# xuhao1/TaichiSLAM

Hardware: AMD Instinct MI355X
Metric: depth-frames/s integrated (640x480->512^3 TSDF) (higher is better)
Workload: dtype f16 storage / f32 + int64 fixed-point arithmetic; 1 GPU; BASELINE configs[1]: single 640x480 u16 depth stream (sphere room r=3 m, 1 deg/frame) -> DenseTSDF 512^3 / 2 cm, recast_step 2, max_ray 5 m; one stream+submap per GPU

## Files before the change

### taichislam_amd/csrc/tsl_integrate.hip

```cpp
#include "tsl_tsdf.hpp"
#include <hip/hip_ext.h>

namespace tsl {

#ifdef TSL_TIMING
#define TSL_T0() const int _wv = (blockIdx.x * (int)blockDim.x + (int)threadIdx.x) >> 6
#define TSL_TICK(F, k) do { long long _n = wall_clock64(); if (lane_id() == 0 && _wv < 16384) (F).dbg[_wv * 16 + (k)] = _n; } while (0)
#else
#define TSL_T0() do {} while (0)
#define TSL_TICK(F, k) do {} while (0)
#endif

#define SCATTER_TILE 4096

struct RayRegs { float pf0, pf1, pf2, d0, d1, d2, P0, P1, P2, w; long long qden; int n; };

__device__ __forceinline__ uint32_t wave_min_u32(uint32_t v)
{
    for (int d = 32; d > 0; d >>= 1) { const uint32_t o = (uint32_t)__shfl_xor((int)v, d); v = o < v ? o : v; }
    return v;
}
__device__ __forceinline__ RayRegs make_ray(const uint4 rec, int n, const FrameParams& P)
{
    RayRegs R;
// ... 426 lines not shown
    if (i < nact) {
        b = F.act_b[i];
        v = F.bhist[b];
        int vq[TSL_NB];
#pragma unroll
        for (int q = 0; q < TSL_NB; ++q) { vq[q] = q < B.n ? B.f[q].bhist[b] : 0; if (vq[q] > 0) tm |= 1 << q; wb += vq[q]; }
        if (wb > unit_max) { tmp = tm; }
        else if (wb > unit_half) {
            int acc = 0;
#pragma unroll
            for (int q = 0; q < TSL_NB; ++q) if ((tm >> q) & 1) { if (2 * acc < wb) { tmu |= 1 << q; wu += vq[q]; } else tmp |= 1 << q; acc += vq[q]; }
        } else { tmu = tm; wu = wb; }
        if (tmu && (tmu & -tmu) == (1 << y)) ucls = plan_class(wu);
        if (((tmp >> y) & 1) && v > 0) { np = (v + psegs - 1) / psegs; pcls = plan_class((v + np - 1) / np); }
    }
    const int off = block_reserve_n(&F.counters[3], v);
    const int s0 = block_reserve_n(&B.f[0].counters[HDR_SLAB], np);
    int p0 = 0, u0 = 0;
    for (int c = 0; c < PLAN_NCLS; ++c) {
        const int q = block_reserve_n(&F.counters[HDR_PARTS + c], pcls == c ? np : 0); if (pcls == c) p0 = q;
        const int u = block_reserve_n(&B.f[0].counters[HDR_UNITS + c], ucls == c ? 1 : 0); if (ucls == c) u0 = u;
    }
    if (i < nact) {
        F.boffset[b] = off;
        F.bnseg[b] = v;
        const int pool = (np || ucls >= 0) ? pool_claim<false>(M, B.p[y]->slot, b) : -1;
        if (ucls >= 0) {
            if (u0 < B.f[0].unit_cap) B.f[0].unit_tab[(size_t)ucls * B.f[0].unit_cap + u0] = make_int4(b, wu, pool, tmu);
            else for (int q = 0; q < B.n; ++q) if ((tm >> q) & 1) frame_fail(M, B.f[q], 2);
        }
        if (np && pool >= 0) {
            if ((tmp & -tmp) == (1 << y)) {
                const int hi = __hip_atomic_fetch_add(&B.f[0].counters[HDR_HEAVY], 1, __ATOMIC_RELAXED, __HIP_MEMORY_SCOPE_AGENT);
                if (hi < B.f[0].max_frame_bricks) B.f[0].heavy_tab[hi] = make_int4(b, pool, tmp, 0);
                else for (int q = 0; q < B.n; ++q) if ((tm >> q) & 1) frame_fail(M, B.f[q], 2);
            }
// ... 546 lines not shown
#pragma unroll
        for (int k = 0; k < VP; ++k) if (changed[k]) {
            tw[l0 + k * 256] = cur[k];
            if ((first[k] >> 16) == 0u) obs[l0 + k * 256] = 1;
        }
    }
}

int check_variant2(tsl_tsdf* m)
{
    TSL_REQUIRE(m->F.max_frame_bricks <= 4096 && m->P.max_steps_f < (float)(1 << SEG_J_BITS) && m->F.max_points < (1 << STG_RAY_BITS) && m->nb3 < (1 << 24) && 3 * m->pcl_bits <= H_BLOCK_SHIFT,
                "variant 2: ray too long / too many points / too many bricks for the segment key (use variant 1)");
    return TSL_OK;
}

int launch_segments(tsl_tsdf* m, const BatchDev& B, const FrameParams* hp, int total, hipStream_t st)
{
    const FrameParams& P = hp[0];
    if (P.variant != 2) return TSL_OK;
    const int iblocks = (int)(((int64_t)total * P.split + 255) / 256);
    prof_begin(m, TSL_K_SEGMENTS, st);
    if (P.group) hipLaunchKernelGGL(k_segments<true>, dim3(iblocks, B.n), dim3(256), 0, st, m->M, B);
    else hipLaunchKernelGGL(k_segments<false>, dim3(iblocks, B.n), dim3(256), 0, st, m->M, B);
    prof_end(m, st);
    int unit_max = m->unit_max <= m->unit_floor ? m->unit_max : std::max(m->unit_floor, (int)((long long)m->unit_max * B.n / TSL_NB));
    int unit_half = std::min(unit_max, m->unit_half <= 2048 ? m->unit_half : std::max(2048, (int)((long long)m->unit_half * B.n / TSL_NB)));
    if (P.seq && m->seq_impl) unit_max = unit_half = 1 << 30;
    prof_begin(m, TSL_K_BIN, st);
    hipLaunchKernelGGL(k_plan, dim3((B.f[0].max_frame_bricks + 255) / 256, B.n), dim3(256), 0, st, m->M, B, m->chunks * m->wg * m->spt, unit_max, unit_half);
    hipLaunchKernelGGL(k_scatter, dim3(256, B.n), dim3(256), 0, st, B);
    prof_end(m, st);
    return TSL_OK;
}

int launch_brick(tsl_tsdf* m, const BatchDev& B, const FrameParams& P, int kind, hipStream_t st, hipEvent_t start, hipEvent_t stop)
{
    const int bg = kind == 2 ? m->pgrid : (B.n <= 2 ? (m->bgrid + 1) / 2 : (kind == 1 ? m->ugrid : m->bgrid));
#define TSL_LAUNCH_IB(TEXV, FD) do { \
        if (m->wg == 512 && m->spt == 2 && !TEXV) hipExtLaunchKernelGGL((k_integrate_batch<false, FD, 512, 2, 4>), dim3((2 * m->ncu * bg + 99) / 100), dim3(512), 0, st, start, stop, 0, m->M, B, kind); \
// ... 41 lines not shown
```

### taichislam_amd/csrc/tsl_tsdf.hip

```cpp
#include "tsl_tsdf.hpp"
#include <rocprim/rocprim.hpp>
#include <algorithm>
#include <cmath>
#include <cstdio>
#include <cstdlib>
#include <cstring>
#include <mutex>

namespace tsl {

static thread_local std::string g_err;
void set_error(const std::string& s) { g_err = s; }

__device__ __forceinline__ uint32_t part1by2_32(uint32_t x)
{
    x &= 0x3ffu;
    x = (x ^ (x << 16)) & 0xff0000ffu;
    x = (x ^ (x << 8)) & 0x0300f00fu;
    x = (x ^ (x << 4)) & 0x030c30c3u;
    x = (x ^ (x << 2)) & 0x09249249u;
    return x;
}
__device__ __forceinline__ uint64_t part1by2_64(uint64_t x)
{
// ... 437 lines not shown
        uint4 v[4];
#pragma unroll
        for (int u = 0; u < 4; ++u) { const int j = i + u * 256; v[u] = j < n ? src[j] : make_uint4(0u, 0u, 0u, 0u); }
#pragma unroll
        for (int u = 0; u < 4; ++u) { const int j = i + u * 256; if (j < n) dst[j] = v[u]; }
    }
}

__global__ void k_set_params(ParamPack PP, SetPtrs S)
{
    if (threadIdx.x == 0) *S.p[blockIdx.x] = PP.p[blockIdx.x];
    S.header[blockIdx.x][threadIdx.x] = 0;
}

template <typename K>
static int enqueue_phase_a(tsl_tsdf* m, const BatchDev& B, const FrameParams* hp, hipStream_t sa)
{
    const int n = B.n;
    int total = 0, tiles = 0, any_points = 0, any_depth = 0;
    for (int q = 0; q < n; ++q) {
        total = hp[q].total > total ? hp[q].total : total;
        const int t = ((hp[q].ww + 15) / 16) * ((hp[q].hh + 15) / 16);
        if (hp[q].points) any_points = 1; else { any_depth = 1; tiles = t > tiles ? t : tiles; }
    }
    if (total <= 0) return TSL_OK;
    const FrameParams& P0 = hp[0];
    const int blocks = (total + 255) / 256;
    prof_begin(m, TSL_K_VOXELIZE, sa);
    if (any_points) hipLaunchKernelGGL(k_voxelize_points<K>, dim3(blocks, n), dim3(256), 0, sa, B);
    if (any_depth) hipLaunchKernelGGL(k_voxelize_depth<K>, dim3(tiles, n), dim3(256), 0, sa, B);
    prof_end(m, sa);
    if (!P0.group) {
        const FrameDev& F = B.f[0];
        prof_begin(m, TSL_K_SORT, sa);
        size_t tb = m->sort_temp_bytes;
        TSL_HIP(rocprim::radix_sort_pairs(m->fset[m->cur * TSL_NB].sort_temp, tb, reinterpret_cast<K*>(F.keys), reinterpret_cast<K*>(F.keys_s), F.vals, F.vals_s, (size_t)total, 0u, (unsigned)(3 * P0.pcl_bits + 1), sa));
        prof_end(m, sa);
        prof_begin(m, TSL_K_RAYS, sa);
        hipLaunchKernelGGL(k_build_rays<K>, dim3(blocks), dim3(256), 0, sa, B.p[0], F, (const K*)reinterpret_cast<K*>(F.keys_s));
        prof_end(m, sa);
    }
    return launch_segments(m, B, hp, total, sa);
}

template <typename K>
static int launch_batch_t(tsl_tsdf* m)
{
    const int n = m->npend;
    if (n == 0) return TSL_OK;
    m->npend = 0;
    (void)hipGetLastError();
    m->last_batch_n = n;
    const int bi = m->cur;
    BatchHost& H = m->batch[bi];
    const bool serial = m->overlap == 0;
    {
        const BatchHost& L = m->batch[(bi + TSL_NBATCH - 1) % TSL_NBATCH];
        if (!L.b_pending || hipEventQuery(L.b_done) == hipSuccess) { m->ramp = 0; ++m->dry_launches; } else if (m->ramp < 1000) ++m->ramp;
        m->shape_hash = (m->shape_hash ^ (uint32_t)n) * 16777619u;
    }
    hipStream_t sa = serial ? m->stream_ : H.st;
    const int ring = (int)(m->batch_seq % TSL_INFLIGHT);
    if (m->ring_upto[ring] > 0) {
        TSL_HIP(hipEventSynchronize(m->ring_ev[ring]));
        if (m->ring_upto[ring] > m->frames_consumed) m->frames_consumed = m->ring_upto[ring];
    }
#ifdef TSL_TEST_HOOKS
    static const bool fault_no_wait = std::getenv("TSL_FAULT_NO_BDONE_WAIT") != nullptr;
#else
    constexpr bool fault_no_wait = false;
#endif
    if (!serial && H.b_pending && !fault_no_wait) TSL_HIP(hipStreamWaitEvent(sa, H.b_done, 0));
    if (!serial && m->esdf_gate_set) {
        TSL_HIP(hipStreamWaitEvent(sa, m->esdf_gate_ev, 0));
        m->esdf_gate_mask |= 1u << (bi % TSL_NSTREAMS);
        if (m->esdf_gate_mask == (1u << TSL_NSTREAMS) - 1u) m->esdf_gate_set = false;
    }
    for (int k = 0; k < m->nproducers; ++k) {
        if (m->producers[k] == sa) continue;
        if (hipStreamQuery(m->producers[k]) == hipSuccess) continue;
        if (!m->in_ev[0]) for (auto& e : m->in_ev) TSL_HIP(hipEventCreateWithFlags(&e, hipEventDisableTiming));
        hipEvent_t e = m->in_ev[m->in_ev_next]; m->in_ev_next = (m->in_ev_next + 1) % 8;
        TSL_HIP(hipEventRecord(e, m->producers[k]));
        TSL_HIP(hipStreamWaitEvent(sa, e, 0));
    }
    m->nproducers = 0;
    BatchDev B; ParamPack PP;
    for (int q = 0; q < n; ++q) { FSet& S = m->fset[bi * TSL_NB + q]; B.f[q] = S.F; B.p[q] = S.Pd; PP.p[q] = m->pend[q]; }
    for (int q = n; q < TSL_NB; ++q) { B.f[q] = B.f[0]; B.p[q] = B.p[0]; PP.p[q] = PP.p[0]; }
    B.n = n;
    SetPtrs SP;
    for (int q = 0; q < TSL_NB; ++q) { SP.p[q] = const_cast<FrameParams*>(B.p[q]); SP.header[q] = reinterpret_cast<int*>(B.f[q].stats); }
    hipLaunchKernelGGL(k_set_params, dim3(n), dim3(64), 0, sa, PP, SP);
    {
        StageCopy C; int most = 0; bool any_host = false;
        for (int q = 0; q < TSL_NB; ++q) {
            FSet& S = m->fset[bi * TSL_NB + q];
            const bool on = q < n;
            C.src[2 * q] = static_cast<const uint4*>(S.pin_dev); C.dst[2 * q] = static_cast<uint4*>(S.stage_in); C.n16[2 * q] = on ? (int)((S.copy_in + 15) / 16) : 0;
            C.src[2 * q + 1] = reinterpret_cast<const uint4*>(static_cast<const char*>(S.pin_dev) + S.copy_tex_off); C.dst[2 * q + 1] = static_cast<uint4*>(S.stage_tex); C.n16[2 * q + 1] = on ? (int)((S.copy_tex + 15) / 16) : 0;
            most = std::max(most, std::max(C.n16[2 * q], C.n16[2 * q + 1]));
            any_host = any_host || C.n16[2 * q] || C.n16[2 * q + 1];
            if (on) { S.copy_in = 0; S.copy_tex = 0; }
        }
        if (any_host) {
            prof_begin(m, TSL_K_VOXELIZE, sa);
            hipLaunchKernelGGL(k_stage_host, dim3(std::min(64, (most + 1023) / 1024), 2 * n), dim3(256), 0, sa, C);
            prof_end(m, sa);
            if (!serial) { TSL_HIP(hipEventRecord(H.c_done, sa)); H.c_recorded = true; }
        }
    }
    if (m->phases & 1) { int rc = enqueue_phase_a<K>(m, B, m->pend, sa); if (rc) return rc; }
    const bool seq_bricks = m->pend[0].seq && m->seq_impl && m->pend[0].variant == 2;
    if (seq_bricks && (m->phases & 1)) { int rc = launch_seq_group(m, B, m->pend, bi, sa); if (rc) return rc; }
    m->frames_issued += n;
    if (!serial) {
        TSL_HIP(hipEventRecord(H.a_done, sa)); H.a_recorded = true;
        TSL_HIP(hipStreamWaitEvent(m->stream_, H.a_done, 0));
    }
    bool any = false; for (int q = 0; q < n; ++q) any = any || m->pend[q].total > 0;
    const bool split = !serial && m->split_launch && (m->phases & 2) && m->pend[0].variant == 2 && !m->pend[0].seq && n > 2 && any;
    if (split) {
        hipEvent_t pa = nullptr, pb = nullptr;
        const bool timed = prof_slot(m, TSL_K_INTEGRATE, 0, &pa, &pb);
        int rc = launch_brick(m, B, m->pend[0], 2, sa, timed ? pa : nullptr, timed ? pb : nullptr);
        if (rc) return rc;
        TSL_HIP(hipEventRecord(H.p_done, sa));
// ... 51 lines not shown
template <int PICK>
static void pick_pixels(uint16_t* __restrict__ dst, const uint16_t* __restrict__ src, int n, int pick)
{
    if (PICK) { for (int i = 0; i < n; ++i) dst[i] = src[(size_t)i * PICK]; }
    else for (int i = 0; i < n; ++i) dst[i] = src[(size_t)i * pick];
}
static int stage_host(tsl_tsdf* m, int si, const void* in, size_t row_bytes, int rows, size_t src_pitch, const void* tex, size_t tex_bytes, void** in_dev, void** tex_dev,
                      int pick = 1)
{
    const int npick = pick > 1 ? (int)(row_bytes / sizeof(uint16_t)) / pick : 0;
    const size_t out_row = pick > 1 ? (size_t)npick * sizeof(uint16_t) : row_bytes;
    const size_t in_bytes = out_row * (size_t)rows;
    FSet& S = m->fset[si];
    BatchHost& H = m->batch[si / TSL_NB];
    if (m->overlap == 0) TSL_HIP(hipStreamSynchronize(m->stream_));
    else if (H.c_recorded) TSL_HIP(hipEventSynchronize(H.c_done));
    const size_t tex_off = (in_bytes + 255) & ~(size_t)255;
    const size_t need = tex_off + ((tex && tex_bytes) ? tex_bytes : 0) + 256;
    if (S.pin_bytes < need) {
        if (S.pin) (void)hipHostFree(S.pin);
        S.pin = nullptr; S.pin_bytes = 0; S.pin_dev = nullptr;
#ifdef TSL_TEST_HOOKS
        static const bool legacy = std::getenv("TSL_PIN_LEGACY") != nullptr;
#else
        constexpr bool legacy = false;
#endif
        TSL_HIP(hipHostMalloc(&S.pin, need + need / 4, legacy ? hipHostMallocMapped : (hipHostMallocMapped | hipHostMallocCoherent)));
        S.pin_bytes = need + need / 4;
        TSL_HIP(hipHostGetDevicePointer(&S.pin_dev, S.pin, 0));
    }
    char* pin = static_cast<char*>(S.pin);
// ... 108 lines not shown
    if (P.variant == 2) { int rc = check_variant2(m); if (rc) return rc; }
    P.input = xyz_dev ? xyz_dev : depth_dev; P.total = total; P.points = xyz_dev ? 1 : 0;
    {
        int lg = 10; while ((1ll << lg) < 2 * (long long)total) ++lg;
        P.hlog2 = lg < m->fset[0].F.hlog2 ? lg : m->fset[0].F.hlog2;
    }
    TSL_REQUIRE(!P.tex || P.variant == 2, "texture integration needs the brick-binned path (variant 2)");
    const int cap = batch_cap(m);
    { int si = 0; int rc = reserve_slot(m, P.points, &si); if (rc) return rc; }
    m->clean = false;
    m->pend_points = P.points;
    m->pend[m->npend] = P;
    m->pend[m->npend].group = (P.group && P.variant == 2) ? 1 : 0;
    m->last_set = m->cur * TSL_NB + m->npend;
    m->npend++;
    if (m->npend >= cap || (cap > 4 && m->ramp < m->ramp_batches && m->npend >= m->ramp_size)) return flush_pending(m);
    if (cap > 1 && m->adaptive) {
        const int last = (m->cur + TSL_NBATCH - 1) % TSL_NBATCH;
        const BatchHost& H = m->batch[last];
        if (!H.a_recorded || hipEventQuery(H.a_done) == hipSuccess) return flush_pending(m);
    }
    return TSL_OK;
}

static int sort_temp_size(tsl_tsdf* m, size_t* bytes)
{
    size_t a = 0, b = 0;
    TSL_HIP(rocprim::radix_sort_pairs(nullptr, a, (uint32_t*)nullptr, (uint32_t*)nullptr, (uint32_t*)nullptr, (uint32_t*)nullptr,
                                      (size_t)m->F.max_points, 0u, 32u, m->stream_));
    TSL_HIP(rocprim::radix_sort_pairs(nullptr, b, (uint64_t*)nullptr, (uint64_t*)nullptr, (uint32_t*)nullptr, (uint32_t*)nullptr,
                                      (size_t)m->F.max_points, 0u, 64u, m->stream_));
// ... 36 lines not shown
{
    int c = 0;
    hipError_t e = hipGetDeviceCount(&c);
    if (e != hipSuccess) { c = 0; }
    if (n) *n = c;
    return TSL_OK;
}

static int init_handle(tsl_tsdf* m, const tsl_tsdf_cfg* cfg, int device)
{
    m->cfg = *cfg; m->device = device; m->bytes = 0;
    (void)hipGetLastError();
    TSL_HIP(hipStreamCreateWithFlags(&m->stream_, hipStreamNonBlocking));
    m->overlap = TSL_NB; m->last_set = 0;
    for (auto& S : m->fset) { S.sort_temp = nullptr; S.header = nullptr; S.Pd = nullptr; S.stage_in = nullptr; S.stage_in_bytes = 0; S.stage_tex = nullptr; S.stage_tex_bytes = 0; S.pin = nullptr; S.pin_bytes = 0; S.pin_dev = nullptr; S.copy_in = S.copy_tex = S.copy_tex_off = 0; }
    for (auto& H : m->batch) { H.st = nullptr; H.a_done = nullptr; H.b_done = nullptr; H.p_done = nullptr; H.c_done = nullptr; H.b_pending = false; H.a_recorded = false; H.c_recorded = false; }
    m->frames_issued = 0; m->frames_consumed = 0; m->batch_seq = 0;
    for (int k = 0; k < TSL_INFLIGHT; ++k) { m->ring_ev[k] = nullptr; m->ring_upto[k] = 0; }
    m->cur = 0; m->npend = 0; m->pend_points = 0; m->deferred_rc = 0;
    const int blk = cfg->num_voxel_per_blk_axis;
    m->N = (int)std::ceil(cfg->map_size_xy / cfg->voxel_scale / (double)blk) * blk;
    m->Nz = (int)std::ceil(cfg->map_size_z / cfg->voxel_scale / (double)blk) * blk;
    TSL_REQUIRE(m->N > 0 && m->Nz > 0 && m->N <= 32768 && m->Nz <= 32768, "tsl_tsdf_create: map extent must fit int16 voxel indices");
    m->nbx = (m->N + 15) / 16; m->nbz = (m->Nz + 15) / 16; m->nb3 = m->nbx * m->nbx * m->nbz;
    m->nsub = cfg->is_global_map ? 1 : (cfg->max_submap_num > 0 ? cfg->max_submap_num : 1);
    m->npose = cfg->max_submap_num > m->nsub ? cfg->max_submap_num : m->nsub;
    {
        int grp = (int)(3.2 * cfg->max_ray_length / (double)blk / cfg->voxel_scale);
        if (grp < 1) grp = 1;
        const int ext = blk * grp;
        int off = -ext / 2; if ((-ext) % 2 != 0) off -= 1;
        m->pcl_lo = off; m->pcl_ext = ext;
        int bits = 1; while ((1 << bits) < ext) ++bits;
        m->pcl_bits = bits;
// ... 10 lines not shown
        P.rvs = best; P.fastdiv = 0;
    }
    P.thr_max = (float)(cfg->max_ray_length * 1000.0); P.thr_min = (float)(cfg->min_ray_length * 1000.0);
    P.max_ray_f = (float)cfg->max_ray_length;
    P.max_steps_f = (float)(cfg->max_ray_length / cfg->voxel_scale);
    P.internal_f = (float)cfg->internal_voxels;
    P.pcl_lo = m->pcl_lo; P.pcl_ext = m->pcl_ext; P.pcl_bits = m->pcl_bits; P.pcl_blk = blk; P.seq = 0;
    P.step = cfg->recast_step; P.same_proj = cfg->color_same_proj;
    m->surf_thres = (float)(cfg->voxel_scale * 1.8);
    m->disp_floor = (float)cfg->disp_floor; m->disp_ceiling = (float)cfg->disp_ceiling;
    m->baseR.assign((size_t)m->npose * 9, 0.0); m->baseT.assign((size_t)m->npose * 3, 0.0);
    m->baseRf.assign((size_t)m->npose * 9, 0.0f); m->baseTf.assign((size_t)m->npose * 3, 0.0f);
    for (int s = 0; s < m->npose; ++s) for (int i = 0; i < 3; ++i) { m->baseR[(size_t)s * 9 + i * 4] = 1.0; m->baseRf[(size_t)s * 9 + i * 4] = 1.0f; }
    std::memset(m->gbaseR, 0, sizeof(m->gbaseR)); std::memset(m->gbaseT, 0, sizeof(m->gbaseT));
    for (int i = 0; i < 3; ++i) m->gbaseR[i * 4] = 1.0;
    m->P.group = 1; m->phases = 3; m->wg = 512; m->spt = 2; m->adaptive = 0; m->ramp_batches = 2; m->ramp_size = 4; m->bgrid = 75; m->ugrid = 75; m->pgrid = 25; m->split_launch = 0; m->chunks = 4; m->unit_max = 1024 * TSL_NB; m->unit_half = 1 << 20; m->unit_floor = 4096; m->batch_gen = 0;
    { hipDeviceProp_t pr; TSL_HIP(hipGetDeviceProperties(&pr, device)); m->ncu = pr.multiProcessorCount > 0 ? pr.multiProcessorCount : 256; }
    m->active = 0; m->variant = 2; m->split = 2; m->semantics = 0; m->seq_impl = 1; m->seq_ready = false; m->seq_bytes0 = 0; m->seq_d = nullptr; m->seq_tuple_cap = 0;
    m->prof_on = false; m->prof_open = false; m->prof_group = false; m->prof_mask = ~0u; std::memset(m->prof_ms, 0, sizeof(m->prof_ms)); std::memset(m->prof_n, 0, sizeof(m->prof_n));
    m->sort_temp = nullptr; m->sort_temp_bytes = 0;
    m->xbuf = nullptr; m->xbuf_bytes = 0; m->mesh_v = m->mesh_n = m->mesh_c = nullptr; m->mesh_count = nullptr; m->mesh_cap = 0; m->mesh_flags = nullptr;
    m->fuse_acc = nullptr; m->fuse_cnt = nullptr; m->fuse_cacc = nullptr; m->fuse_dirty = false; m->mrg_nunion = -1;
    m->esdf = nullptr; m->esdf_par = nullptr; m->esdf_ok = nullptr; m->esdf_mode = 0; m->esdf_grid = 0; m->fuse_direct = false; m->merge_exchange = 0; m->mrg_racc = m->mrg_rcnt = m->mrg_rec = nullptr; m->mrg_racc_bytes = m->mrg_rcnt_bytes = m->mrg_rec_bytes = 0; m->esdf_orphans = 0; m->esdf_last = nullptr; m->esdf_in = nullptr; m->esdf_read = nullptr; m->esdf_overlap = true; m->esdf_ctr_idx = 0; for (int k = 0; k < 2; ++k) { m->fseq_keys[k] = m->fseq_vals[k] = nullptr; m->fseq_bytes[k] = m->fseq_vbytes[k] = 0; } m->fseq_temp = nullptr; m->fseq_tbytes = 0; m->fseq_ctr = nullptr; m->esdf_gate = nullptr; m->esdf_gate_ev = nullptr; m->esdf_gate_set = false; m->esdf_gate_mask = 0; m->esdf_valid = false; m->esdf_force_full = false; m->pose_dev = nullptr;

    MapDev& M = m->M; std::memset(&M, 0, sizeof(M));
    M.N = m->N; M.Nz = m->Nz; M.nbx = m->nbx; M.nbz = m->nbz; M.nb3 = m->nb3; M.nsub = m->nsub; M.hN = m->N / 2; M.hNz = m->Nz / 2;
    int64_t want = cfg->max_bricks > 0 ? cfg->max_bricks : 32768 * (int64_t)(m->nsub > 4 ? 4 : (m->nsub > 1 ? m->nsub : 1));
    const int64_t all = (int64_t)m->nsub * m->nb3;
    if (want > all) want = all;
    M.max_bricks = (int)want;
    int rc;
// ... 161 lines not shown
    TSL_HIP(hipMemcpyAsync(m->h_ints, dev, sizeof(int), hipMemcpyDeviceToHost, ms(m)));
    TSL_HIP(hipStreamSynchronize(ms(m)));
    *out = m->h_ints[0];
    return take_deferred(m);
}
static int check_dev_err(tsl_tsdf* m) { (void)ms(m); return take_dev_err(m); }
int tsl_tsdf_get_option(tsl_tsdf* m, const char* name, int* value)
{
    TSL_REQUIRE(m && name && value, "null");
    if (!std::strcmp(name, "group")) { *value = m->P.group; return TSL_OK; }
    if (!std::strcmp(name, "esdf_mode")) { *value = m->esdf_mode; return TSL_OK; }
    if (!std::strcmp(name, "fuse_window_misses")) { return read_int(m, m->M.pool_top + 2, value); }
    if (!std::strcmp(name, "esdf_orphans")) { int rc = esdf_finish(m); if (rc) return rc; *value = (int)m->esdf_orphans; return TSL_OK; }
    if (!std::strcmp(name, "semantics")) { *value = m->semantics; return TSL_OK; }
    if (!std::strcmp(name, "seq_impl")) { *value = m->seq_impl; return TSL_OK; }
    if (!std::strcmp(name, "last_heavy_bricks") || !std::strcmp(name, "last_slab_slots")) {
        TSL_REQUIRE(m->scratch_ready, "nothing integrated yet");
        int rc = tsl_tsdf_sync(m); if (rc) return rc;
        const int bi = (m->cur + TSL_NBATCH - 1) % TSL_NBATCH;
        int v[40];
        TSL_HIP(hipMemcpy(v, m->fset[bi * TSL_NB].F.counters, sizeof(v), hipMemcpyDeviceToHost));
        *value = name[5] == 'h' ? v[14] : v[13];
        return TSL_OK;
    }
    if (!std::strcmp(name, "seq_longest_run")) {
        TSL_REQUIRE(m->scratch_ready, "nothing integrated yet");
        int rc = tsl_tsdf_sync(m); if (rc) return rc;
        const int bi = (m->cur + TSL_NBATCH - 1) % TSL_NBATCH;
        long long sum = 0;
        for (int q = 0; q < m->last_batch_n; ++q) { int v[40]; TSL_HIP(hipMemcpy(v, m->fset[bi * TSL_NB + q].F.counters, sizeof(v), hipMemcpyDeviceToHost)); sum += (unsigned)v[31]; }
        *value = (int)(sum > 0x7fffffffll ? 0x7fffffffll : sum);
        return TSL_OK;
    }
    if (!std::strcmp(name, "seq_long_voxels")) {
        TSL_REQUIRE(m->scratch_ready, "nothing integrated yet");
        int rc = tsl_tsdf_sync(m); if (rc) return rc;
        const int bi = (m->cur + TSL_NBATCH - 1) % TSL_NBATCH;
// ... 399 lines not shown
        return TSL_OK;
    }
    if (!std::strcmp(name, "fastdiv")) { if (value == 0) m->P.fastdiv = 0; return TSL_OK; }
    if (!std::strcmp(name, "mesh_gather")) { m->mesh_gather = value != 0; return TSL_OK; }
    if (!std::strcmp(name, "esdf_full")) { m->esdf_force_full = value != 0; return TSL_OK; }
    if (!std::strcmp(name, "esdf_mode")) { TSL_REQUIRE(value == 0 || value == 1, "esdf_mode: 0 = regional recompute (default), 1 = raise / lower wavefront with parent directions"); int rc = esdf_finish(m); if (rc) return rc; m->esdf_mode = value; m->esdf_valid = false; return TSL_OK; }
    if (!std::strcmp(name, "esdf_round_cap")) { m->esdf_round_cap = value; return TSL_OK; }
    if (!std::strcmp(name, "merge_exchange")) { TSL_REQUIRE(value == 0 || value == 1, "merge_exchange: 0 = all-reduce of the packed sums, 1 = reduce-scatter + all-gather of finalised voxels"); m->merge_exchange = value; return TSL_OK; }
    if (!std::strcmp(name, "fuse_direct")) { m->fuse_direct = value != 0; return TSL_OK; }
    if (!std::strcmp(name, "esdf_grid")) { TSL_REQUIRE(value >= 0, "esdf_grid: workgroups of a relaxation round (0 = four per CU)"); m->esdf_grid = value; return TSL_OK; }
    if (!std::strcmp(name, "esdf_overlap")) { int rc = esdf_finish(m); if (rc) return rc; m->esdf_overlap = value != 0; return TSL_OK; }
    if (!std::strcmp(name, "unit")) { TSL_REQUIRE(value >= 0 && value <= (1 << 20), "unit must be 0..2^20 segments"); int rc = tsl_tsdf_sync(m); if (rc) return rc; m->unit_max = value; return TSL_OK; }
    if (!std::strcmp(name, "unit_floor")) { TSL_REQUIRE(value >= 0 && value <= (1 << 20), "unit_floor must be 0..2^20 segments"); int rc = tsl_tsdf_sync(m); if (rc) return rc; m->unit_floor = value; return TSL_OK; }
    if (!std::strcmp(name, "unit_half")) { TSL_REQUIRE(value >= 0 && value <= (1 << 20), "unit_half must be 0..2^20 segments"); int rc = tsl_tsdf_sync(m); if (rc) return rc; m->unit_half = value; return TSL_OK; }
    if (!std::strcmp(name, "chunks")) { TSL_REQUIRE(value >= 1 && value <= 8, "chunks must be 1..8"); int rc = tsl_tsdf_sync(m); if (rc) return rc; m->chunks = value; return TSL_OK; }
    if (!std::strcmp(name, "adaptive")) { m->adaptive = value != 0; return TSL_OK; }
    if (!std::strcmp(name, "ramp_size")) { TSL_REQUIRE(value >= 1 && value <= TSL_NB, "ramp_size must be 1..8 frames"); m->ramp_size = value; return TSL_OK; }
    if (!std::strcmp(name, "ramp")) { TSL_REQUIRE(value >= 0 && value <= 16, "ramp must be 0..16 half batches"); m->ramp_batches = value; return TSL_OK; }
    if (!std::strcmp(name, "ugrid") || !std::strcmp(name, "pgrid")) { TSL_REQUIRE(value >= 5 && value <= 200, "ugrid / pgrid must be 5..200 (percent of the resident workgroup slots)"); { int rc = tsl_tsdf_sync(m); if (rc) return rc; } (name[0] == 'u' ? m->ugrid : m->pgrid) = value; return TSL_OK; }
    if (!std::strcmp(name, "split_launch")) { TSL_REQUIRE(value == 0 || value == 1, "split_launch must be 0 or 1"); { int rc = tsl_tsdf_sync(m); if (rc) return rc; } m->split_launch = value; return TSL_OK; }
    if (!std::strcmp(name, "bgrid")) { TSL_REQUIRE(value >= 10 && value <= 200, "bgrid must be 10..200 (percent of the resident workgroup slots)"); { int rc = tsl_tsdf_sync(m); if (rc) return rc; } m->bgrid = value; return TSL_OK; }
    if (!std::strcmp(name, "spt")) { TSL_REQUIRE(value == 2 || value == 4, "spt must be 2 or 4"); { int rc = tsl_tsdf_sync(m); if (rc) return rc; } m->spt = value; return TSL_OK; }
    if (!std::strcmp(name, "wg")) { TSL_REQUIRE(value == 256 || value == 512, "wg must be 256 or 512"); { int rc = tsl_tsdf_sync(m); if (rc) return rc; } m->wg = value; return TSL_OK; }
    if (!std::strcmp(name, "phases")) { int rc = tsl_tsdf_sync(m); if (rc) return rc; m->phases = value & 3; return TSL_OK; }
    if (!std::strcmp(name, "overlap")) { int rc = tsl_tsdf_sync(m); if (rc) return rc; m->overlap = value < 0 ? 0 : (value > TSL_NB ? TSL_NB : value); for (auto& H : m->batch) H.b_pending = false; return TSL_OK; }
    if (!std::strcmp(name, "split")) { TSL_REQUIRE(value >= 1 && value <= 64 && (64 % value) == 0, "split must divide 64"); m->split = value; return TSL_OK; }
    set_error("unknown option"); return TSL_ERR_ARG;
}

}
// ... 1 lines not shown
```

### taichislam_amd/csrc/tsl_tsdf.hpp

```cpp
#pragma once
#include "tsl_common.hpp"

namespace tsl {

struct FrameParams {
    float R[9], T[3];
    float fx, fy, cx, cy;
    float fxc, fyc, cxc, cyc;
    float vs;
    float rvs; int fastdiv;
    float thr_max, thr_min;
    float max_ray_f;
    float max_steps_f;
    float internal_f;
    int   pcl_lo, pcl_ext, pcl_bits;
    int   step, hh, ww, H, W;
    int   rstride;
    int   cstride;
    int   th, tw, tex, same_proj;
    int   slot;
    int   variant, split;
    int   group;
    int   seq, pcl_blk;
    int   hlog2;
// ... 143 lines not shown
#define TSL_NB 8
#define TSL_NBATCH 3
#define TSL_NSTREAMS 3
#define TSL_NSETS (TSL_NB * TSL_NBATCH)
struct FSet {
    FrameDev F; void* sort_temp; void* header; size_t header_bytes;
    void* stage_in; size_t stage_in_bytes; void* stage_tex; size_t stage_tex_bytes;
    void* pin; size_t pin_bytes; void* pin_dev;
    size_t copy_in, copy_tex, copy_tex_off;
    FrameParams* Pd;
    std::vector<void*> owned;
};
struct BatchDev { FrameDev f[TSL_NB]; const FrameParams* p[TSL_NB]; int n; };
struct ParamPack { FrameParams p[TSL_NB]; };
struct SetPtrs { FrameParams* p[TSL_NB]; int* header[TSL_NB]; };
struct BatchHost { hipStream_t st; hipEvent_t a_done, b_done, p_done, c_done; bool b_pending, a_recorded, c_recorded; };
struct StageCopy { const uint4* src[2 * TSL_NB]; uint4* dst[2 * TSL_NB]; int n16[2 * TSL_NB]; };
#define TSL_INFLIGHT 8

int fuse_submaps_sequential(tsl_tsdf* g, tsl_tsdf* sub, const float* pose_dev, int nsrc);
int esdf_finish(tsl_tsdf* m);
int esdf_read_check(tsl_tsdf* m, const char* who);
void esdf_release(tsl_tsdf* m);
struct FrontierState;
void frontier_release(tsl_tsdf* m);
struct GainState;
void gain_release(tsl_tsdf* m);
struct MeshIdxState;
void mesh_indexed_release(tsl_tsdf* m);
struct NavState;
void nav_release(tsl_tsdf* m);
// ... 4 lines not shown
void nav_field3_release(tsl_tsdf* m);
}

#define TSL_ESDF_SLOTS 4
struct EsdfSlot { hipEvent_t ev; int* host; int rounds; tsl_esdf_stats st; };
struct tsl_tsdf {
    tsl_tsdf_cfg cfg;
    int device;
    hipStream_t stream_;
    tsl::FSet fset[TSL_NSETS]; tsl::BatchHost batch[TSL_NBATCH]; hipStream_t copy_st;
    int overlap;
    int cur, npend, pend_points; tsl::FrameParams pend[TSL_NB]; int deferred_rc;
    int64_t frames_issued, frames_consumed;
    int64_t batch_seq; hipEvent_t ring_ev[TSL_INFLIGHT]; int64_t ring_upto[TSL_INFLIGHT];
    int last_set, last_batch_n;
    hipStream_t producers[4]; int nproducers;
    hipEvent_t in_ev[8]; int in_ev_next;
    bool scratch_ready;
    int N, Nz, nbx, nbz, nb3, nsub, npose;
    int pcl_lo, pcl_ext, pcl_bits;
    tsl::MapDev M;
    tsl::FrameDev F;
    tsl::FrameParams P;
    std::vector<double> baseR, baseT;
    std::vector<float> baseRf, baseTf;
    double gbaseR[9], gbaseT[3];
    int active;
    float surf_thres, disp_floor, disp_ceiling;
    void* sort_temp; size_t sort_temp_bytes;
    tsl_frame_stats* h_stats;
// ... 36 lines not shown
    tsl::NavFieldState* nav_field;
    tsl::NavTerrainState* nav_terrain;
    tsl::NavFieldState* nav_field3;
};

namespace tsl {
int  grow(void** p, size_t* have, size_t need);
hipStream_t ms(tsl_tsdf* m);
int  flush_pending(tsl_tsdf* m);
void prof_begin(tsl_tsdf* m, int kid, hipStream_t st = nullptr, int count = 1);
void prof_end(tsl_tsdf* m, hipStream_t st = nullptr);
bool prof_slot(tsl_tsdf* m, int kid, int count, hipEvent_t* a, hipEvent_t* b);
void convert_pose(const double* Rb, const double* Tb, const double* R, const double* T, float* outR, float* outT);
int  dev_alloc(tsl_tsdf* m, void** p, size_t bytes, int fill);
int  check_variant2(tsl_tsdf* m);
int  launch_segments(tsl_tsdf* m, const BatchDev& B, const FrameParams* hp, int total, hipStream_t st);
int  launch_apply(tsl_tsdf* m, FSet& S, int total);
int  launch_apply_batch(tsl_tsdf* m, const BatchDev& B, const FrameParams& P, hipEvent_t start = nullptr, hipEvent_t stop = nullptr);
int  launch_brick(tsl_tsdf* m, const BatchDev& B, const FrameParams& P, int kind, hipStream_t st, hipEvent_t start, hipEvent_t stop);
int  launch_slab_apply(tsl_tsdf* m, const BatchDev& B, const FrameParams& P);
int  launch_seq_group(tsl_tsdf* m, const BatchDev& B, const FrameParams* hp, int bi, hipStream_t st);
int  launch_seq_apply(tsl_tsdf* m, const BatchDev& B, const FrameParams& P, int bi);
void seq_release(tsl_tsdf* m);
int  order_before(tsl_tsdf* m, hipStream_t user, hipStream_t q);
int  order_after(tsl_tsdf* m, hipStream_t user, hipStream_t q);
int  nav_edt_launch(tsl_tsdf* m, hipStream_t q, int N, int B, int R, int flags, int cost_unknown, const uint8_t* cls, uint8_t* g, const uint8_t* lut, uint16_t* d2,
                    uint8_t* cost);
int  seq_prepare(tsl_tsdf* m);
int  selftest_seqdiv(unsigned long long* bad_dev);
int  seq_verify_report(tsl_tsdf* m, int* out, int cap);
int  launch_apply_sequential(tsl_tsdf* m, const BatchDev& B, const FrameParams& P);
// ... 2 lines not shown
```

Measured before the change: 34170 frames/s.

## Batch plan counter reservations and add early phase-A issue with dry-start ramping

k_plan now reserves all slab, part and unit counters with one wave-scan pass and a single atomic per counter, replacing repeated block reservations. Host batching gains an optional early issue of voxelize work for partial frame groups, a dry-start ramp flag that flushes smaller first batches, a larger default ramp size, and an optional stream-priority mode. The aim is less launch/atomic overhead and earlier overlap of host staging with GPU work. It adds more host-side state and ordering logic, with some risk around partially staged batches.

```diff
diff --git a/taichislam_amd/csrc/tsl_integrate.hip b/taichislam_amd/csrc/tsl_integrate.hip
--- a/taichislam_amd/csrc/tsl_integrate.hip
+++ b/taichislam_amd/csrc/tsl_integrate.hip
@@ -464,12 +464,35 @@
         if (tmu && (tmu & -tmu) == (1 << y)) ucls = plan_class(wu);
         if (((tmp >> y) & 1) && v > 0) { np = (v + psegs - 1) / psegs; pcls = plan_class((v + np - 1) / np); }
     }
-    const int off = block_reserve_n(&F.counters[3], v);
-    const int s0 = block_reserve_n(&B.f[0].counters[HDR_SLAB], np);
-    int p0 = 0, u0 = 0;
-    for (int c = 0; c < PLAN_NCLS; ++c) {
-        const int q = block_reserve_n(&F.counters[HDR_PARTS + c], pcls == c ? np : 0); if (pcls == c) p0 = q;
-        const int u = block_reserve_n(&B.f[0].counters[HDR_UNITS + c], ucls == c ? 1 : 0); if (ucls == c) u0 = u;
+    enum { PLAN_NCTR = 2 + 2 * PLAN_NCLS };
+    __shared__ int s_tot[4][PLAN_NCTR];
+    __shared__ int s_base[PLAN_NCTR];
+    int val[PLAN_NCTR], inc[PLAN_NCTR];
+    val[0] = v; val[1] = np;
+#pragma unroll
+    for (int c = 0; c < PLAN_NCLS; ++c) { val[2 + c] = pcls == c ? np : 0; val[2 + PLAN_NCLS + c] = ucls == c ? 1 : 0; }
+    const int lane = lane_id(), wid = threadIdx.x >> 6;
+#pragma unroll
+    for (int k = 0; k < PLAN_NCTR; ++k) {
+        int x = val[k];
+        for (int d = 1; d < 64; d <<= 1) { const int o = __shfl_up(x, d); if (lane >= d) x += o; }
+        inc[k] = x;
+        if (lane == 63) s_tot[wid][k] = x;
+    }
+    __syncthreads();
+    if (threadIdx.x < PLAN_NCTR) {
+        const int k = threadIdx.x;
+        const int tot = s_tot[0][k] + s_tot[1][k] + s_tot[2][k] + s_tot[3][k];
+        int* const ctr = k == 0 ? &F.counters[3] : (k == 1 ? &B.f[0].counters[HDR_SLAB] : (k < 2 + PLAN_NCLS ? &F.counters[HDR_PARTS + k - 2] : &B.f[0].counters[HDR_UNITS + k - 2 - PLAN_NCLS]));
+        s_base[k] = tot ? __hip_atomic_fetch_add(ctr, tot, __ATOMIC_RELAXED, __HIP_MEMORY_SCOPE_AGENT) : 0;
+    }
+    __syncthreads();
+    int off = 0, s0 = 0, p0 = 0, u0 = 0;
+#pragma unroll
+    for (int k = 0; k < PLAN_NCTR; ++k) {
+        int o = s_base[k] + inc[k] - val[k];
+        for (int w = 0; w < wid; ++w) o += s_tot[w][k];
+        if (k == 0) off = o; else if (k == 1) s0 = o; else if (k < 2 + PLAN_NCLS) { if (pcls == k - 2) p0 = o; } else if (ucls == k - 2 - PLAN_NCLS) u0 = o;
     }
     if (i < nact) {
         F.boffset[b] = off;
@@ -1046,15 +1069,18 @@
     return TSL_OK;
 }
 
-int launch_segments(tsl_tsdf* m, const BatchDev& B, const FrameParams* hp, int total, hipStream_t st)
+int launch_segments(tsl_tsdf* m, const BatchDev& B, const FrameParams* hp, int total, hipStream_t st, int parts)
 {
     const FrameParams& P = hp[0];
     if (P.variant != 2) return TSL_OK;
-    const int iblocks = (int)(((int64_t)total * P.split + 255) / 256);
-    prof_begin(m, TSL_K_SEGMENTS, st);
-    if (P.group) hipLaunchKernelGGL(k_segments<true>, dim3(iblocks, B.n), dim3(256), 0, st, m->M, B);
-    else hipLaunchKernelGGL(k_segments<false>, dim3(iblocks, B.n), dim3(256), 0, st, m->M, B);
-    prof_end(m, st);
+    if (parts & 1) {
+        const int iblocks = (int)(((int64_t)total * P.split + 255) / 256);
+        prof_begin(m, TSL_K_SEGMENTS, st);
+        if (P.group) hipLaunchKernelGGL(k_segments<true>, dim3(iblocks, B.n), dim3(256), 0, st, m->M, B);
+        else hipLaunchKernelGGL(k_segments<false>, dim3(iblocks, B.n), dim3(256), 0, st, m->M, B);
+        prof_end(m, st);
+    }
+    if (!(parts & 2)) return TSL_OK;
     int unit_max = m->unit_max <= m->unit_floor ? m->unit_max : std::max(m->unit_floor, (int)((long long)m->unit_max * B.n / TSL_NB));
     int unit_half = std::min(unit_max, m->unit_half <= 2048 ? m->unit_half : std::max(2048, (int)((long long)m->unit_half * B.n / TSL_NB)));
     if (P.seq && m->seq_impl) unit_max = unit_half = 1 << 30;
diff --git a/taichislam_amd/csrc/tsl_tsdf.hip b/taichislam_amd/csrc/tsl_tsdf.hip
--- a/taichislam_amd/csrc/tsl_tsdf.hip
+++ b/taichislam_amd/csrc/tsl_tsdf.hip
@@ -475,7 +475,7 @@
 }
 
 template <typename K>
-static int enqueue_phase_a(tsl_tsdf* m, const BatchDev& B, const FrameParams* hp, hipStream_t sa)
+static int enqueue_phase_a(tsl_tsdf* m, const BatchDev& B, const FrameParams* hp, hipStream_t sa, int parts = 3)
 {
     const int n = B.n;
     int total = 0, tiles = 0, any_points = 0, any_depth = 0;
@@ -487,11 +487,13 @@
     if (total <= 0) return TSL_OK;
     const FrameParams& P0 = hp[0];
     const int blocks = (total + 255) / 256;
-    prof_begin(m, TSL_K_VOXELIZE, sa);
-    if (any_points) hipLaunchKernelGGL(k_voxelize_points<K>, dim3(blocks, n), dim3(256), 0, sa, B);
-    if (any_depth) hipLaunchKernelGGL(k_voxelize_depth<K>, dim3(tiles, n), dim3(256), 0, sa, B);
-    prof_end(m, sa);
-    if (!P0.group) {
+    if (parts & 1) {
+        prof_begin(m, TSL_K_VOXELIZE, sa);
+        if (any_points) hipLaunchKernelGGL(k_voxelize_points<K>, dim3(blocks, n), dim3(256), 0, sa, B);
+        if (any_depth) hipLaunchKernelGGL(k_voxelize_depth<K>, dim3(tiles, n), dim3(256), 0, sa, B);
+        prof_end(m, sa);
+    }
+    if (!P0.group && parts == 3) {
         const FrameDev& F = B.f[0];
         prof_begin(m, TSL_K_SORT, sa);
         size_t tb = m->sort_temp_bytes;
@@ -501,42 +503,27 @@
         hipLaunchKernelGGL(k_build_rays<K>, dim3(blocks), dim3(256), 0, sa, B.p[0], F, (const K*)reinterpret_cast<K*>(F.keys_s));
         prof_end(m, sa);
     }
-    return launch_segments(m, B, hp, total, sa);
-}
-
-template <typename K>
-static int launch_batch_t(tsl_tsdf* m)
-{
-    const int n = m->npend;
-    if (n == 0) return TSL_OK;
-    m->npend = 0;
-    (void)hipGetLastError();
-    m->last_batch_n = n;
-    const int bi = m->cur;
+    return launch_segments(m, B, hp, total, sa, parts);
+}
+
+static int open_slot(tsl_tsdf* m, int bi, hipStream_t sa)
+{
     BatchHost& H = m->batch[bi];
-    const bool serial = m->overlap == 0;
-    {
-        const BatchHost& L = m->batch[(bi + TSL_NBATCH - 1) % TSL_NBATCH];
-        if (!L.b_pending || hipEventQuery(L.b_done) == hipSuccess) { m->ramp = 0; ++m->dry_launches; } else if (m->ramp < 1000) ++m->ramp;
-        m->shape_hash = (m->shape_hash ^ (uint32_t)n) * 16777619u;
-    }
-    hipStream_t sa = serial ? m->stream_ : H.st;
-    const int ring = (int)(m->batch_seq % TSL_INFLIGHT);
-    if (m->ring_upto[ring] > 0) {
-        TSL_HIP(hipEventSynchronize(m->ring_ev[ring]));
-        if (m->ring_upto[ring] > m->frames_consumed) m->frames_consumed = m->ring_upto[ring];
-    }
 #ifdef TSL_TEST_HOOKS
     static const bool fault_no_wait = std::getenv("TSL_FAULT_NO_BDONE_WAIT") != nullptr;
 #else
     constexpr bool fault_no_wait = false;
 #endif
-    if (!serial && H.b_pending && !fault_no_wait) TSL_HIP(hipStreamWaitEvent(sa, H.b_done, 0));
-    if (!serial && m->esdf_gate_set) {
+    if (H.b_pending && !fault_no_wait) TSL_HIP(hipStreamWaitEvent(sa, H.b_done, 0));
+    if (m->esdf_gate_set) {
         TSL_HIP(hipStreamWaitEvent(sa, m->esdf_gate_ev, 0));
         m->esdf_gate_mask |= 1u << (bi % TSL_NSTREAMS);
         if (m->esdf_gate_mask == (1u << TSL_NSTREAMS) - 1u) m->esdf_gate_set = false;
     }
+    return TSL_OK;
+}
+static int wait_producers(tsl_tsdf* m, hipStream_t sa)
+{
     for (int k = 0; k < m->nproducers; ++k) {
         if (m->producers[k] == sa) continue;
         if (hipStreamQuery(m->producers[k]) == hipSuccess) continue;
@@ -546,8 +533,15 @@
         TSL_HIP(hipStreamWaitEvent(sa, e, 0));
     }
     m->nproducers = 0;
-    BatchDev B; ParamPack PP;
-    for (int q = 0; q < n; ++q) { FSet& S = m->fset[bi * TSL_NB + q]; B.f[q] = S.F; B.p[q] = S.Pd; PP.p[q] = m->pend[q]; }
+    return TSL_OK;
+}
+template <typename K>
+static int issue_frames(tsl_tsdf* m, int bi, int q0, int q1, hipStream_t sa, bool serial, int parts, BatchDev& B)
+{
+    BatchHost& H = m->batch[bi];
+    const int n = q1 - q0;
+    ParamPack PP;
+    for (int q = 0; q < n; ++q) { FSet& S = m->fset[bi * TSL_NB + q0 + q]; B.f[q] = S.F; B.p[q] = S.Pd; PP.p[q] = m->pend[q0 + q]; }
     for (int q = n; q < TSL_NB; ++q) { B.f[q] = B.f[0]; B.p[q] = B.p[0]; PP.p[q] = PP.p[0]; }
     B.n = n;
     SetPtrs SP;
@@ -556,8 +550,8 @@
     {
         StageCopy C; int most = 0; bool any_host = false;
         for (int q = 0; q < TSL_NB; ++q) {
-            FSet& S = m->fset[bi * TSL_NB + q];
             const bool on = q < n;
+            FSet& S = m->fset[bi * TSL_NB + (on ? q0 + q : q0)];
             C.src[2 * q] = static_cast<const uint4*>(S.pin_dev); C.dst[2 * q] = static_cast<uint4*>(S.stage_in); C.n16[2 * q] = on ? (int)((S.copy_in + 15) / 16) : 0;
             C.src[2 * q + 1] = reinterpret_cast<const uint4*>(static_cast<const char*>(S.pin_dev) + S.copy_tex_off); C.dst[2 * q + 1] = static_cast<uint4*>(S.stage_tex); C.n16[2 * q + 1] = on ? (int)((S.copy_tex + 15) / 16) : 0;
             most = std::max(most, std::max(C.n16[2 * q], C.n16[2 * q + 1]));
@@ -568,10 +562,89 @@
             prof_begin(m, TSL_K_VOXELIZE, sa);
             hipLaunchKernelGGL(k_stage_host, dim3(std::min(64, (most + 1023) / 1024), 2 * n), dim3(256), 0, sa, C);
             prof_end(m, sa);
-            if (!serial) { TSL_HIP(hipEventRecord(H.c_done, sa)); H.c_recorded = true; }
-        }
-    }
-    if (m->phases & 1) { int rc = enqueue_phase_a<K>(m, B, m->pend, sa); if (rc) return rc; }
+            if (!serial) { TSL_HIP(hipEventRecord(H.c_done, sa)); H.c_recorded = true; H.c_open = parts == 1; }
+        }
+    }
+    if (m->phases & 1) { int rc = enqueue_phase_a<K>(m, B, m->pend + q0, sa, parts); if (rc) return rc; }
+    return TSL_OK;
+}
+
+static bool early_eligible(const tsl_tsdf* m)
+{
+    const FrameParams& P0 = m->pend[0];
+    return m->early_a != 0 && m->overlap > 1 && !m->split_launch && m->phases == 3 && P0.variant == 2 && P0.group && !P0.seq;
+}
+template <typename K>
+static int issue_early_t(tsl_tsdf* m)
+{
+    const int bi = m->cur;
+    hipStream_t sa = m->batch[bi].st;
+    (void)hipGetLastError();
+    if (!m->early_open) { int rc = open_slot(m, bi, sa); if (rc) return rc; m->early_open = true; }
+    { int rc = wait_producers(m, sa); if (rc) return rc; }
+    BatchDev B;
+    { int rc = issue_frames<K>(m, bi, m->early_n, m->npend, sa, false, 1, B); if (rc) return rc; }
+    m->early_n = m->npend; ++m->early_groups_n;
+    TSL_HIP(hipGetLastError());
+    return TSL_OK;
+}
+static int early_groups(tsl_tsdf* m)
+{
+    if (!early_eligible(m)) return TSL_OK;
+    int g = m->early_a;
+    if (g < 0) {
+        if (m->npend == 1) { const BatchHost& L = m->batch[(m->cur + TSL_NBATCH - 1) % TSL_NBATCH]; m->early_dry = m->ramp_first || !L.b_pending || hipEventQuery(L.b_done) == hipSuccess; }
+        g = (m->early_dry || m->ramp + 1 < m->early_ramp) ? m->early_g_ramp : m->early_g_steady;
+        if (g == 0) return TSL_OK;
+    }
+    if (m->npend - m->early_n < g) return TSL_OK;
+    const FrameParams keep = m->P;
+    const int rc = m->pcl_bits <= 10 ? issue_early_t<uint32_t>(m) : issue_early_t<uint64_t>(m);
+    m->P = keep;
+    if (rc) {
+        m->npend = 0; m->early_n = 0; m->early_open = false; m->nproducers = 0; m->batch[m->cur].c_open = false;
+        if (!m->deferred_rc) m->deferred_rc = rc;
+    }
+    return rc;
+}
+
+template <typename K>
+static int launch_batch_t(tsl_tsdf* m)
+{
+    const int n = m->npend;
+    if (n == 0) return TSL_OK;
+    m->npend = 0;
+    const int early = m->early_n; const bool opened = m->early_open;
+    m->early_n = 0; m->early_open = false;
+    (void)hipGetLastError();
+    m->last_batch_n = n;
+    const int bi = m->cur;
+    BatchHost& H = m->batch[bi];
+    const bool serial = m->overlap == 0;
+    {
+        const BatchHost& L = m->batch[(bi + TSL_NBATCH - 1) % TSL_NBATCH];
+        if (!L.b_pending || hipEventQuery(L.b_done) == hipSuccess) { m->ramp = (m->ramp_first && m->ramp_batches > 0) ? 1 : 0; ++m->dry_launches; } else if (m->ramp < 1000) ++m->ramp;
+        m->ramp_first = false;
+        m->shape_hash = (m->shape_hash ^ (uint32_t)n) * 16777619u;
+    }
+    hipStream_t sa = serial ? m->stream_ : H.st;
+    const int ring = (int)(m->batch_seq % TSL_INFLIGHT);
+    if (m->ring_upto[ring] > 0) {
+        TSL_HIP(hipEventSynchronize(m->ring_ev[ring]));
+        if (m->ring_upto[ring] > m->frames_consumed) m->frames_consumed = m->ring_upto[ring];
+    }
+    if (!serial && !opened) { int rc = open_slot(m, bi, sa); if (rc) return rc; }
+    { int rc = wait_producers(m, sa); if (rc) return rc; }
+    H.c_open = false;
+    BatchDev B;
+    if (early == 0) { int rc = issue_frames<K>(m, bi, 0, n, sa, serial, 3, B); if (rc) return rc; }
+    else {
+        if (early < n) { int rc = issue_frames<K>(m, bi, early, n, sa, serial, 1, B); if (rc) return rc; H.c_open = false; }
+        for (int q = 0; q < n; ++q) { FSet& S = m->fset[bi * TSL_NB + q]; B.f[q] = S.F; B.p[q] = S.Pd; }
+        for (int q = n; q < TSL_NB; ++q) { B.f[q] = B.f[0]; B.p[q] = B.p[0]; }
+        B.n = n;
+        { int rc = enqueue_phase_a<K>(m, B, m->pend, sa, 2); if (rc) return rc; }
+    }
     const bool seq_bricks = m->pend[0].seq && m->seq_impl && m->pend[0].variant == 2;
     if (seq_bricks && (m->phases & 1)) { int rc = launch_seq_group(m, B, m->pend, bi, sa); if (rc) return rc; }
     m->frames_issued += n;
@@ -653,7 +726,7 @@
     FSet& S = m->fset[si];
     BatchHost& H = m->batch[si / TSL_NB];
     if (m->overlap == 0) TSL_HIP(hipStreamSynchronize(m->stream_));
-    else if (H.c_recorded) TSL_HIP(hipEventSynchronize(H.c_done));
+    else if (H.c_recorded && !H.c_open) TSL_HIP(hipEventSynchronize(H.c_done));
     const size_t tex_off = (in_bytes + 255) & ~(size_t)255;
     const size_t need = tex_off + ((tex && tex_bytes) ? tex_bytes : 0) + 256;
     if (S.pin_bytes < need) {
@@ -792,7 +865,15 @@
     m->pend[m->npend].group = (P.group && P.variant == 2) ? 1 : 0;
     m->last_set = m->cur * TSL_NB + m->npend;
     m->npend++;
-    if (m->npend >= cap || (cap > 4 && m->ramp < m->ramp_batches && m->npend >= m->ramp_size)) return flush_pending(m);
+    if (m->npend == 1) {
+        m->ramp_first = false;
+        if (cap > 4 && m->dry_first && m->ramp_batches > 0 && m->ramp >= m->ramp_batches) {
+            const BatchHost& L = m->batch[(m->cur + TSL_NBATCH - 1) % TSL_NBATCH];
+            m->ramp_first = !L.b_pending || hipEventQuery(L.b_done) == hipSuccess;
+        }
+    }
+    if (m->npend >= cap || (cap > 4 && (m->ramp < m->ramp_batches || m->ramp_first) && m->npend >= m->ramp_size)) return flush_pending(m);
+    if (cap > 1 && !m->adaptive) return early_groups(m);
     if (cap > 1 && m->adaptive) {
         const int last = (m->cur + TSL_NBATCH - 1) % TSL_NBATCH;
         const BatchHost& H = m->batch[last];
@@ -859,10 +940,12 @@
     TSL_HIP(hipStreamCreateWithFlags(&m->stream_, hipStreamNonBlocking));
     m->overlap = TSL_NB; m->last_set = 0;
     for (auto& S : m->fset) { S.sort_temp = nullptr; S.header = nullptr; S.Pd = nullptr; S.stage_in = nullptr; S.stage_in_bytes = 0; S.stage_tex = nullptr; S.stage_tex_bytes = 0; S.pin = nullptr; S.pin_bytes = 0; S.pin_dev = nullptr; S.copy_in = S.copy_tex = S.copy_tex_off = 0; }
-    for (auto& H : m->batch) { H.st = nullptr; H.a_done = nullptr; H.b_done = nullptr; H.p_done = nullptr; H.c_done = nullptr; H.b_pending = false; H.a_recorded = false; H.c_recorded = false; }
+    for (auto& H : m->batch) { H.st = nullptr; H.a_done = nullptr; H.b_done = nullptr; H.p_done = nullptr; H.c_done = nullptr; H.b_pending = false; H.a_recorded = false; H.c_recorded = false; H.c_open = false; }
     m->frames_issued = 0; m->frames_consumed = 0; m->batch_seq = 0;
     for (int k = 0; k < TSL_INFLIGHT; ++k) { m->ring_ev[k] = nullptr; m->ring_upto[k] = 0; }
     m->cur = 0; m->npend = 0; m->pend_points = 0; m->deferred_rc = 0;
+    m->ramp_first = false; m->dry_first = 1;
+    m->early_a = 0; m->early_ramp = 4; m->early_n = 0; m->early_open = false; m->early_dry = true; m->early_groups_n = 0; m->early_g_ramp = 2; m->early_g_steady = 4; m->stream_prio = 0;
     const int blk = cfg->num_voxel_per_blk_axis;
     m->N = (int)std::ceil(cfg->map_size_xy / cfg->voxel_scale / (double)blk) * blk;
     m->Nz = (int)std::ceil(cfg->map_size_z / cfg->voxel_scale / (double)blk) * blk;
@@ -903,7 +986,7 @@
     for (int s = 0; s < m->npose; ++s) for (int i = 0; i < 3; ++i) { m->baseR[(size_t)s * 9 + i * 4] = 1.0; m->baseRf[(size_t)s * 9 + i * 4] = 1.0f; }
     std::memset(m->gbaseR, 0, sizeof(m->gbaseR)); std::memset(m->gbaseT, 0, sizeof(m->gbaseT));
     for (int i = 0; i < 3; ++i) m->gbaseR[i * 4] = 1.0;
-    m->P.group = 1; m->phases = 3; m->wg = 512; m->spt = 2; m->adaptive = 0; m->ramp_batches = 2; m->ramp_size = 4; m->bgrid = 75; m->ugrid = 75; m->pgrid = 25; m->split_launch = 0; m->chunks = 4; m->unit_max = 1024 * TSL_NB; m->unit_half = 1 << 20; m->unit_floor = 4096; m->batch_gen = 0;
+    m->P.group = 1; m->phases = 3; m->wg = 512; m->spt = 2; m->adaptive = 0; m->ramp_batches = 2; m->ramp_size = 6; m->bgrid = 75; m->ugrid = 75; m->pgrid = 25; m->split_launch = 0; m->chunks = 4; m->unit_max = 1024 * TSL_NB; m->unit_half = 1 << 20; m->unit_floor = 4096; m->batch_gen = 0;
     { hipDeviceProp_t pr; TSL_HIP(hipGetDeviceProperties(&pr, device)); m->ncu = pr.multiProcessorCount > 0 ? pr.multiProcessorCount : 256; }
     m->active = 0; m->variant = 2; m->split = 2; m->semantics = 0; m->seq_impl = 1; m->seq_ready = false; m->seq_bytes0 = 0; m->seq_d = nullptr; m->seq_tuple_cap = 0;
     m->prof_on = false; m->prof_open = false; m->prof_group = false; m->prof_mask = ~0u; std::memset(m->prof_ms, 0, sizeof(m->prof_ms)); std::memset(m->prof_n, 0, sizeof(m->prof_n));
@@ -1095,13 +1178,17 @@
     if (!std::strcmp(name, "esdf_orphans")) { int rc = esdf_finish(m); if (rc) return rc; *value = (int)m->esdf_orphans; return TSL_OK; }
     if (!std::strcmp(name, "semantics")) { *value = m->semantics; return TSL_OK; }
     if (!std::strcmp(name, "seq_impl")) { *value = m->seq_impl; return TSL_OK; }
-    if (!std::strcmp(name, "last_heavy_bricks") || !std::strcmp(name, "last_slab_slots")) {
+    if (!std::strcmp(name, "early_a")) { *value = m->early_a; return TSL_OK; }
+    if (!std::strcmp(name, "dry_first")) { *value = m->dry_first; return TSL_OK; }
+    if (!std::strcmp(name, "early_groups")) { *value = m->early_groups_n; return TSL_OK; }
+    if (!std::strcmp(name, "stream_prio")) { *value = m->stream_prio; return TSL_OK; }
+    if (!std::strcmp(name, "last_heavy_bricks") || !std::strcmp(name, "last_slab_slots") || !std::strcmp(name, "last_units")) {
         TSL_REQUIRE(m->scratch_ready, "nothing integrated yet");
         int rc = tsl_tsdf_sync(m); if (rc) return rc;
         const int bi = (m->cur + TSL_NBATCH - 1) % TSL_NBATCH;
         int v[40];
         TSL_HIP(hipMemcpy(v, m->fset[bi * TSL_NB].F.counters, sizeof(v), hipMemcpyDeviceToHost));
-        *value = name[5] == 'h' ? v[14] : v[13];
+        *value = name[5] == 'h' ? v[HDR_HEAVY] : (name[5] == 's' ? v[HDR_SLAB] : v[HDR_UNITS] + v[HDR_UNITS + 1] + v[HDR_UNITS + 2] + v[HDR_UNITS + 3]);
         return TSL_OK;
     }
     if (!std::strcmp(name, "seq_longest_run")) {
@@ -1531,6 +1618,40 @@
     if (!std::strcmp(name, "unit_floor")) { TSL_REQUIRE(value >= 0 && value <= (1 << 20), "unit_floor must be 0..2^20 segments"); int rc = tsl_tsdf_sync(m); if (rc) return rc; m->unit_floor = value; return TSL_OK; }
     if (!std::strcmp(name, "unit_half")) { TSL_REQUIRE(value >= 0 && value <= (1 << 20), "unit_half must be 0..2^20 segments"); int rc = tsl_tsdf_sync(m); if (rc) return rc; m->unit_half = value; return TSL_OK; }
     if (!std::strcmp(name, "chunks")) { TSL_REQUIRE(value >= 1 && value <= 8, "chunks must be 1..8"); int rc = tsl_tsdf_sync(m); if (rc) return rc; m->chunks = value; return TSL_OK; }
+    if (!std::strcmp(name, "early_a")) { TSL_REQUIRE(value >= -1 && value <= TSL_NB, "early_a must be -1 (by regime), 0 (off) or 1..8 frames per group"); int rc = tsl_tsdf_sync(m); if (rc) return rc; m->early_a = value; return TSL_OK; }
+    if (!std::strcmp(name, "stream_prio")) {
+        TSL_REQUIRE(value == 0 || value == 1, "stream_prio must be 0 or 1");
+        int rc = tsl_tsdf_sync(m); if (rc) return rc;
+        rc = esdf_finish(m); if (rc) return rc;
+        if (value == m->stream_prio) return TSL_OK;
+        TSL_HIP(hipSetDevice(m->device));
+        int least = 0, greatest = 0;
+        TSL_HIP(hipDeviceGetStreamPriorityRange(&least, &greatest));
+        TSL_HIP(hipStreamSynchronize(m->stream_));
+        hipStream_t fresh[1 + TSL_NSTREAMS] = {};
+        for (int k = 0; k <= TSL_NSTREAMS; ++k) {
+            const hipError_t e = value ? hipStreamCreateWithPriority(&fresh[k], hipStreamNonBlocking, k == 0 ? greatest : least) : hipStreamCreateWithFlags(&fresh[k], hipStreamNonBlocking);
+            if (e != hipSuccess) { for (int j = 0; j < k; ++j) (void)hipStreamDestroy(fresh[j]); TSL_HIP(e); }
+        }
+        (void)hipStreamDestroy(m->stream_); m->stream_ = fresh[0];
+        for (int bi = 0; bi < TSL_NSTREAMS; ++bi) { (void)hipStreamDestroy(m->batch[bi].st); m->batch[bi].st = fresh[1 + bi]; }
+        for (int bi = TSL_NSTREAMS; bi < TSL_NBATCH; ++bi) m->batch[bi].st = m->batch[bi % TSL_NSTREAMS].st;
+        m->nproducers = 0;
+        if (m->scratch_ready) {
+            int* const word = m->num_particles + 2;
+            TSL_HIP(hipMemsetAsync(word, 0, 4, m->stream_));
+            TSL_HIP(hipStreamSynchronize(m->stream_));
+            for (int bi = 0; bi < TSL_NSTREAMS; ++bi) { TSL_HIP(hipMemsetAsync(word, 0, 4, m->batch[bi].st)); TSL_HIP(hipStreamSynchronize(m->batch[bi].st)); }
+        }
+        m->stream_prio = value;
+        return TSL_OK;
+    }
+    if (!std::strcmp(name, "early_g_ramp") || !std::strcmp(name, "early_g_steady")) {
+        TSL_REQUIRE(value >= 0 && value <= TSL_NB, "early_g_ramp / early_g_steady must be 0..8 frames");
+        (name[8] == 'r' ? m->early_g_ramp : m->early_g_steady) = value; return TSL_OK;
+    }
+    if (!std::strcmp(name, "early_ramp")) { TSL_REQUIRE(value >= 0 && value <= 1000, "early_ramp must be 0..1000 batches"); m->early_ramp = value; return TSL_OK; }
+    if (!std::strcmp(name, "dry_first")) { m->dry_first = value != 0; return TSL_OK; }
     if (!std::strcmp(name, "adaptive")) { m->adaptive = value != 0; return TSL_OK; }
     if (!std::strcmp(name, "ramp_size")) { TSL_REQUIRE(value >= 1 && value <= TSL_NB, "ramp_size must be 1..8 frames"); m->ramp_size = value; return TSL_OK; }
     if (!std::strcmp(name, "ramp")) { TSL_REQUIRE(value >= 0 && value <= 16, "ramp must be 0..16 half batches"); m->ramp_batches = value; return TSL_OK; }
diff --git a/taichislam_amd/csrc/tsl_tsdf.hpp b/taichislam_amd/csrc/tsl_tsdf.hpp
--- a/taichislam_amd/csrc/tsl_tsdf.hpp
+++ b/taichislam_amd/csrc/tsl_tsdf.hpp
@@ -181,7 +181,7 @@
 struct BatchDev { FrameDev f[TSL_NB]; const FrameParams* p[TSL_NB]; int n; };
 struct ParamPack { FrameParams p[TSL_NB]; };
 struct SetPtrs { FrameParams* p[TSL_NB]; int* header[TSL_NB]; };
-struct BatchHost { hipStream_t st; hipEvent_t a_done, b_done, p_done, c_done; bool b_pending, a_recorded, c_recorded; };
+struct BatchHost { hipStream_t st; hipEvent_t a_done, b_done, p_done, c_done; bool b_pending, a_recorded, c_recorded, c_open; };
 struct StageCopy { const uint4* src[2 * TSL_NB]; uint4* dst[2 * TSL_NB]; int n16[2 * TSL_NB]; };
 #define TSL_INFLIGHT 8
 
@@ -216,6 +216,9 @@
     int64_t frames_issued, frames_consumed;
     int64_t batch_seq; hipEvent_t ring_ev[TSL_INFLIGHT]; int64_t ring_upto[TSL_INFLIGHT];
     int last_set, last_batch_n;
+    int early_a, early_ramp, early_g_ramp, early_g_steady, early_n, early_groups_n; bool early_open, early_dry;
+    bool ramp_first; int dry_first;
+    int stream_prio;
     hipStream_t producers[4]; int nproducers;
     hipEvent_t in_ev[8]; int in_ev_next;
     bool scratch_ready;
@@ -282,7 +285,7 @@
 void convert_pose(const double* Rb, const double* Tb, const double* R, const double* T, float* outR, float* outT);
 int  dev_alloc(tsl_tsdf* m, void** p, size_t bytes, int fill);
 int  check_variant2(tsl_tsdf* m);
-int  launch_segments(tsl_tsdf* m, const BatchDev& B, const FrameParams* hp, int total, hipStream_t st);
+int  launch_segments(tsl_tsdf* m, const BatchDev& B, const FrameParams* hp, int total, hipStream_t st, int parts = 3);
 int  launch_apply(tsl_tsdf* m, FSet& S, int total);
 int  launch_apply_batch(tsl_tsdf* m, const BatchDev& B, const FrameParams& P, hipEvent_t start = nullptr, hipEvent_t stop = nullptr);
 int  launch_brick(tsl_tsdf* m, const BatchDev& B, const FrameParams& P, int kind, hipStream_t st, hipEvent_t start, hipEvent_t stop);
```

Result: no change. 34150 frames/s (-0.0%).
